# rendeirolab/stainx

Hardware: AMD Instinct MI355X
Metric: megapixels/sec Macenko transform, 64x3x512x512 fp32; max-abs vs torch CPU (higher is better)
Workload: dtype f32; 1 GPU; Macenko reference-mode transform, 64x3x512x512 fp32 per GPU (BASELINE configs[1]); tiles_per_gpu=64, height=512, width=512, input_batches_rotated=2, parallelism=tiles sharded over 1 GPU(s), no collective

## Files before the change

### stainx_amd/csrc/macenko_twopass.hpp

```cpp
#pragma once

namespace sx {
namespace macenko {

constexpr int kPriorSweeps = 4;
constexpr int kPriorUnitsMax = kGroupThreads / 4 * kPriorSweeps;
constexpr int kQueue2 = 512;
constexpr float kSpecSigmasConc = 5.0f, kSpecThresholdScale = 1.0f;
constexpr float kSpecSigmas = 5.0f;
constexpr float kSpecEffFar = 2.0f, kSpecEffNear = 1.0f;
__device__ __forceinline__ float spec_eff(const Geometry& g) { return g.prior_step_q16 >= (8u << 16) ? g.spec_eff_far : g.spec_eff_near; }
constexpr float kSpecKw = 0.10f, kSpecKx = 1.3e-3f;
constexpr float kSpecRot = 0.30f;
constexpr uint32_t kSpecSlow = 1u, kSpecHazard = 2u;
constexpr int kMaxSegments = 256;

constexpr int kRowBelowA = 0, kRowAboveA = 1, kRowBelowB = 2, kRowAboveB = 3, kRowConc = 4, kRowW = 8;
struct alignas(128) PriorRecord {
    float a0[3], a1[3], an[3];
    float rows[16][4];
    float kw, kx;
    float cmax[4];
    int32_t mode;
    int32_t min_first;
// ... 2 lines not shown

struct alignas(64) FusedTile {
    uint32_t a_done;
    uint32_t s_done;
    uint32_t ncand[kSlots];
    uint32_t pad[10];
};
constexpr int kXcds = 8;
struct alignas(64) FusedQueue {
    uint32_t ticket;
    uint32_t pad[15];
};
struct FusedSched {
    FusedQueue queue[kXcds];
};
static_assert(sizeof(FusedTile) == kFusedTileBytes && sizeof(FusedSched) <= kFusedSchedBytes, "workspace layout");


typedef unsigned int sx_u4 __attribute__((ext_vector_type(4)));
__device__ __forceinline__ uint32_t ld_agent(const uint32_t* p) { return __hip_atomic_load(p, __ATOMIC_RELAXED, __HIP_MEMORY_SCOPE_AGENT); }
__device__ __forceinline__ int32_t ld_agent(const int32_t* p) { return __hip_atomic_load(p, __ATOMIC_RELAXED, __HIP_MEMORY_SCOPE_AGENT); }
__device__ __forceinline__ float ld_agent(const float* p) { return __uint_as_float(__hip_atomic_load(reinterpret_cast<const uint32_t*>(p), __ATOMIC_RELAXED, __HIP_MEMORY_SCOPE_AGENT)); }
__device__ __forceinline__ double ld_agent(const double* p) {
    return __longlong_as_double((long long)__hip_atomic_load(reinterpret_cast<const unsigned long long*>(p), __ATOMIC_RELAXED, __HIP_MEMORY_SCOPE_AGENT));
}
__device__ __forceinline__ void st_agent(uint32_t* p, uint32_t v) { __hip_atomic_store(p, v, __ATOMIC_RELAXED, __HIP_MEMORY_SCOPE_AGENT); }
__device__ __forceinline__ void st_agent(float* p, float v) { __hip_atomic_store(reinterpret_cast<uint32_t*>(p), __float_as_uint(v), __ATOMIC_RELAXED, __HIP_MEMORY_SCOPE_AGENT); }
__device__ __forceinline__ void st_agent(double* p, double v) {
    __hip_atomic_store(reinterpret_cast<unsigned long long*>(p), (unsigned long long)__double_as_longlong(v), __ATOMIC_RELAXED, __HIP_MEMORY_SCOPE_AGENT);
}
__device__ __forceinline__ void drain_stores() { asm volatile("s_waitcnt vmcnt(0)" ::: "memory"); }

constexpr int kPriorBins = 2048;
constexpr float kOpenExponent = 30.0f;
constexpr float kOpenNear = 16.0f;
struct alignas(16) PriorScratch {
    double red[kGroupThreads / kWave][kPartial];
    double mom[kMoments];
    uint32_t hist[4][kPriorBins];
    uint32_t od16[kPriorSweeps][6][kGroupThreads];
    uint32_t n_kept, n_all, hazard, r_max;
    float frame[9];
    float bdir[4][2];
    float bkey[4], blevel[4];
    float cthr[4];
    uint32_t cmax[4];
    uint32_t open;
};

__device__ __forceinline__ uint32_t prior_pick_bin(const uint32_t* hist, uint32_t rank) {
    constexpr int kPer = kPriorBins / kWave;
    static_assert(kPer <= kWave, "second level: one bin per lane");
    const int lane = (int)lane_id();
    uint32_t mine = 0;
#pragma unroll 8
    for (int i = 0; i < kPer; ++i) mine += hist[kPer * lane + i];
    const uint32_t incl = wave_scan_u32(mine);
    const uint64_t over = __ballot(incl > rank);
    const int owner = over ? (__ffsll((long long)over) - 1) : (kWave - 1);
    const uint32_t r = rank - (uint32_t)__builtin_amdgcn_readlane((int)(incl - mine), owner);
    const uint32_t h = lane < kPer ? hist[kPer * owner + lane] : 0u;
    const uint32_t incl2 = wave_scan_u32(h);
    const uint64_t over2 = __ballot(lane < kPer && incl2 > r);
    const int sub = over2 ? (__ffsll((long long)over2) - 1) : (kPer - 1);
    return (uint32_t)(kPer * owner + sub);
}

__device__ __forceinline__ float wave_total_f32(float x) {
    auto step = [](float v, auto mover) { return v + __uint_as_float(mover(__float_as_uint(v))); };
    x = step(x, [](uint32_t b) { return dpp_move<0x111, 0xF>(0u, b); });
    x = step(x, [](uint32_t b) { return dpp_move<0x112, 0xF>(0u, b); });
    x = step(x, [](uint32_t b) { return dpp_move<0x114, 0xF>(0u, b); });
    x = step(x, [](uint32_t b) { return dpp_move<0x118, 0xF>(0u, b); });
    x = step(x, [](uint32_t b) { return dpp_move<0x142, 0xA>(0u, b); });
    x = step(x, [](uint32_t b) { return dpp_move<0x143, 0xC>(0u, b); });
    return x;
}

// ... 20 lines not shown
}
template <typename T>
__device__ __forceinline__ void prior_densities(const float (&u)[3][4], float (&od)[4][3]) {
#pragma unroll
    for (int i = 0; i < 4; ++i)
#pragma unroll
        for (int c = 0; c < 3; ++c) od[i][c] = optical_density<T>(u[c][i]);
}

template <typename T, bool kVec, bool kInter>
__global__ __launch_bounds__(kGroupThreads) void prior_kernel(const T* __restrict__ images, Geometry g, Workspace ws) {
    __shared__ PriorScratch sh;
    const int tile = blockIdx.x, tid = threadIdx.x, wave = tid / kWave;
    const uint32_t lane = lane_id();
    GroupState& st = ws.state[tile];
    PriorRecord* pr = &ws.prior[tile];
    const T* img = images + (int64_t)tile * 3 * g.pixels;
    SX_STAMP(st, 0);
    if (tid < kSlots) {
        put(&st.ncand[tid], 0u);
        put(&st.below[tid], 0u);
        put(&st.ncand_seen[tid], 0u);
        put(&st.over_count[tid], 0u);
    }
    if (tid < 2) put(&st.phi_pub[tid], 0ull);
    if ((g.fused || g.dense) && tid < (int)(sizeof(FusedTile) / 4)) put(reinterpret_cast<uint32_t*>(&ws.ftile[tile]) + tid, 0u);
    if (g.fused && tile == 0 && tid >= 32 && tid < 32 + kXcds) put(&ws.fsched->queue[tid - 32].ticket, 0u);
    if (tid == 0) {
        put(&st.fell_back, 0u);
        put(&st.spec, 0u);
        sh.n_kept = sh.n_all = sh.hazard = sh.open = sh.r_max = 0;
        sh.cmax[0] = sh.cmax[1] = sh.cmax[2] = sh.cmax[3] = 0;
    }
    for (int i = tid; i < 4 * kPriorBins; i += kGroupThreads) (&sh.hist[0][0])[i] = 0;

    {
        float m[kPartial];
#pragma unroll
        for (int k = 0; k < kPartial; ++k) m[k] = 0.0f;
        float raw[kPriorSweeps][3][4];
        bool have_quad[kPriorSweeps];
#pragma unroll
        for (int s = 0; s < kPriorSweeps; ++s) have_quad[s] = prior_fetch<T, kVec, kInter>(img, g, s, raw[s]);
#pragma unroll
        for (int s = 0; s < kPriorSweeps; ++s) {
            float od[4][3];
            prior_densities<T>(raw[s], od);
            const bool have = have_quad[s];
#pragma unroll
            for (int q = 0; q < 6; ++q) {
                const int e = 2 * q;
                typedef __fp16 fp16x2 __attribute__((ext_vector_type(2)));
                const fp16x2 h = __builtin_amdgcn_cvt_pkrtz(od[e / 3][e % 3], od[(e + 1) / 3][(e + 1) % 3]);
                sh.od16[s][q][tid] = __builtin_bit_cast(uint32_t, h);
            }
#pragma unroll
            for (int i = 0; i < 4; ++i) {
                const float* o = od[i];
                const float keep = (have && od_selected(o, false)) ? 1.0f : 0.0f;
                const float k0 = keep * o[0], k1 = keep * o[1], k2 = keep * o[2];
                m[0] += keep;
                m[1] += k0;
                m[2] += k1;
                m[3] += k2;
                m[4] = fmaf(k0, o[0], m[4]);
                m[5] = fmaf(k0, o[1], m[5]);
                m[6] = fmaf(k0, o[2], m[6]);
// ... 73 lines not shown
            if (have) have_bits |= 1u << s;
#pragma unroll
            for (int i = 0; i < 4; ++i) {
                const float* o = od[i];
                t0[s][i] = fmaf(o[2], fr[2], fmaf(o[1], fr[1], o[0] * fr[0]));
                t1[s][i] = fmaf(o[2], fr[5], fmaf(o[1], fr[4], o[0] * fr[3]));
                if (have) {
                    r_max = fmaxf(r_max, fabsf(t0[s][i]) + fabsf(t1[s][i]));
                    if (i == s) ++all;
                    if (od_selected(o, false)) {
                        if (!(t1[s][i] - 0.05f * fabsf(t0[s][i]) > 0.0f)) haz = 1;
                        if (i == s) {
                            ++cnt;
                            sub_kept |= 1u << s;
                        }
                    }
                }
            }
        }
        cnt = wave_total_u32(cnt);
        all = wave_total_u32(all);
        const uint32_t rm = wave_max_u32(__float_as_uint(r_max));
        const uint64_t hz = __ballot(haz != 0);
        if (lane == 0) {
            if (cnt) atomicAdd(&sh.n_kept, cnt);
            atomicAdd(&sh.n_all, all);
            atomicMax(&sh.r_max, rm);
            if (hz) atomicOr(&sh.hazard, 1u);
        }
#pragma unroll
        for (int s = 0; s < kPriorSweeps; ++s)
            if ((sub_kept >> s) & 1u) {
                const float d = diamond_angle(t1[s][s], t0[s][s]);
                atomicAdd(&sh.hist[0][min((uint32_t)fmaxf(d * (float)(kPriorBins / 2), 0.0f), (uint32_t)(kPriorBins - 1))], 1u);
            }
    }
    __syncthreads();
    SX_STAMP(st, 4);
    if (sh.hazard) {
        give_up();
        return;
    }
    const int mv = (int)sh.n_kept, ms = (int)sh.n_all;
    if (wave < 4) {
        const float f = wave < 2 ? 0.01f : 0.99f;
        const float n_eff = fmaxf((float)mv * (spec_eff(g) / 4.0f), 4.0f);
        const float sd = sqrtf(f * (1.0f - f) / n_eff);
        const bool upper = (wave & 1) != 0;
        const float level = upper ? f + g.spec_sigmas * sd : f - g.spec_sigmas * sd;
        const bool open = mv < 16 || (upper ? level >= 1.0f : level <= 0.0f);
        const float pos = fminf(fmaxf(level, 0.0f), 1.0f) * (float)max(mv - 1, 0);
        const uint32_t rank = (uint32_t)min(max((int)(upper ? ceilf(pos) : floorf(pos)), 0), max(mv - 1, 0));
        const uint32_t b = prior_pick_bin(sh.hist[0], rank);
        if (lane == 0) {
            sh.bkey[wave] = upper ? (float)(b + 1) * (2.0f / kPriorBins) : (float)b * (2.0f / kPriorBins);
            sh.blevel[wave] = fminf(fmaxf(level, 0.0f), 1.0f) * n_eff;
            if (open) atomicOr(&sh.open, 1u << wave);
        }
    }
    __syncthreads();
    if (tid < 4) {
        const bool upper = (tid & 1) != 0, open = ((sh.open >> tid) & 1u) != 0, partner_open = ((sh.open >> (tid ^ 1)) & 1u) != 0;
        float d = sh.bkey[tid];
        if (open) {
            const float other = sh.bkey[tid ^ 1];
            const float n_eff = fmaxf((float)mv * (spec_eff(g) / 4.0f), 4.0f);
            const float m_near = upper ? n_eff - sh.blevel[tid ^ 1] : sh.blevel[tid ^ 1];
            const bool tight = !partner_open && m_near >= kOpenNear;
            const float w = fminf(fmaxf((kOpenExponent - 0.01f * n_eff) / fmaxf(m_near, 1.0f), 0.25f), 1.0f);
            d = !tight ? (upper ? 1.98f : 0.02f) : (upper ? d + w * fmaxf(d - other, 0.0f) + 2.0f / kPriorBins : d - w * fmaxf(other - d, 0.0f) - 2.0f / kPriorBins);
        }
        d = fminf(fmaxf(d, 0.02f), 1.98f);
        float c, s;
        direction_from_key(float_key(d), c, s);
        sh.bdir[tid][0] = c;
        sh.bdir[tid][1] = s;
    }
    __syncthreads();
    SX_STAMP(st, 5);
    float bd[4][2];
#pragma unroll
    for (int q = 0; q < 4; ++q) {
        bd[q][0] = sh.bdir[q][0];
        bd[q][1] = sh.bdir[q][1];
    }
    const float lo_c = bd[0][0] + bd[1][0], lo_s = bd[0][1] + bd[1][1], hi_c = bd[2][0] + bd[3][0], hi_s = bd[2][1] + bd[3][1];
    const bool min_first = (fr[0] * lo_c + fr[3] * lo_s) * __builtin_amdgcn_rsqf(lo_c * lo_c + lo_s * lo_s) > (fr[0] * hi_c + fr[3] * hi_s) * __builtin_amdgcn_rsqf(hi_c * hi_c + hi_s * hi_s);
    float cu[4][2];
    {
        const int slot_perp_high = min_first ? 0 : 1, slot_perp_low = 1 - slot_perp_high;
#pragma unroll
        for (int e = 0; e < 2; ++e) {
            cu[2 * slot_perp_high + e][0] = bd[2 + e][1];
            cu[2 * slot_perp_high + e][1] = -bd[2 + e][0];
            cu[2 * slot_perp_low + e][0] = -bd[e][1];
            cu[2 * slot_perp_low + e][1] = bd[e][0];
        }
    }
    const float r_max = __uint_as_float(sh.r_max);
    const float c_scale = r_max > 0.0f ? (float)kPriorBins / r_max : 0.0f;
    for (int i = tid; i < kPriorBins; i += kGroupThreads) sh.hist[0][i] = 0;
    __syncthreads();
#pragma unroll
    for (int q = 0; q < 4; ++q) {
        float k_max = 0.0f;
#pragma unroll
        for (int s = 0; s < kPriorSweeps; ++s)
            if ((have_bits >> s) & 1u) {
                const float k = fmaf(cu[q][0], t0[s][s], cu[q][1] * t1[s][s]);
                k_max = fmaxf(k_max, k);
                atomicAdd(&sh.hist[q][min((uint32_t)fmaxf(k * c_scale, 0.0f), (uint32_t)(kPriorBins - 1))], 1u);
            }
        const uint32_t km = wave_max_u32(__float_as_uint(k_max));
        if (lane == 0) atomicMax(&sh.cmax[q], km);
    }
    __syncthreads();
    SX_STAMP(st, 6);
    if (wave < 4) {
        const float n_eff = fmaxf((float)ms * (spec_eff(g) / 4.0f), 4.0f);
        const float level = 0.99f - g.spec_sigmas_conc * sqrtf(0.99f * 0.01f / n_eff);
        const uint32_t rank = (uint32_t)max((int)floorf(fmaxf(level, 0.0f) * (float)max(ms - 1, 0)), 0);
        const uint32_t b = prior_pick_bin(sh.hist[wave], rank);
        if (lane == 0) sh.cthr[wave] = (level > 0.0f && b > 0) ? g.spec_tscale * (float)b * (r_max / (float)kPriorBins) : -__builtin_huge_valf();
    }
    __syncthreads();
    if (tid < 9) {
        const float* a0 = &sh.frame[0];
        const float* a1 = &sh.frame[3];
        const float* an = &sh.frame[6];
        const uint32_t open = sh.open;
        float row[4] = {0.0f, 0.0f, 0.0f, 0.0f};
#pragma unroll
        for (int q = 0; q < 4; ++q) {
            if (tid == q && ((open >> q) & 1u) == 0) {
#pragma unroll
                for (int c = 0; c < 3; ++c) row[c] = bd[q][0] * a1[c] - bd[q][1] * a0[c];
            }
            if (tid == kRowConc + q) {
#pragma unroll
                for (int c = 0; c < 3; ++c) row[c] = cu[q][0] * a0[c] + cu[q][1] * a1[c];
                row[3] = sh.cthr[q] > -1e30f ? -sh.cthr[q] : 60000.0f;
            }
        }
        if (tid == kRowW) {
#pragma unroll
            for (int c = 0; c < 3; ++c) row[c] = an[c];
        }
#pragma unroll
        for (int c = 0; c < 4; ++c) put(&pr->rows[tid][c], __half2float(__float2half_rn(row[c])));
    } else if (tid < 16) {
#pragma unroll
        for (int c = 0; c < 4; ++c) put(&pr->rows[tid][c], 0.0f);
    }
    if (tid == 0) {
#pragma unroll
        for (int i = 0; i < 3; ++i) {
            put(&pr->a0[i], sh.frame[i]);
            put(&pr->a1[i], sh.frame[3 + i]);
            put(&pr->an[i], sh.frame[6 + i]);
        }
        put(&pr->kw, g.spec_kw);
        put(&pr->kx, kSpecKx);
#pragma unroll
        for (int q = 0; q < 4; ++q) put(&pr->cmax[q], __uint_as_float(sh.cmax[q]));
        put(&pr->mode, 0);
        put(&pr->min_first, min_first ? 1 : 0);
        put(&pr->open, sh.open);
    }
    SX_STAMP(st, 7);
}

template <int TPB> struct PassAScratch {
    StatsScratch<TPB> stats;
    uint32_t queue[TPB / kWave][4][kQueue2];
    uint32_t below[2];
};

__device__ __forceinline__ void write_records(const uint32_t (*__restrict__ queue)[kQueue2], uint32_t n, uint32_t (&have)[kSlots], float* __restrict__ cand_tile, const Geometry& g, uint32_t seg_base, uint32_t* __restrict__ over_count) {
    const uint32_t cap2 = g.cap2, seg_cap = g.seg_cap, over_base = (uint32_t)g.n_seg * g.seg_cap;
    for (uint32_t i0 = 0; i0 < n; i0 += kWave) {
        const uint32_t i = i0 + lane_id();
        uint4 rec = make_uint4(0u, 0u, 0u, 0u);
        if (i < n) rec = make_uint4(queue[0][i], queue[1][i], queue[2][i], queue[3][i]);
#pragma unroll
        for (int s = 0; s < kSlots; ++s) {
            const bool has = ((rec.w >> s) & 1u) != 0;
            const uint64_t mask = __builtin_amdgcn_ballot_w64(has);
// ... 253 lines not shown
    }
    double kept_total = 0.0;
#pragma unroll
    for (int w = 0; w < TPB / kWave; ++w) kept_total += ss->red[w][0];
    if (__builtin_expect(kept_total < 3.0, 0)) {
        if (!tile_has_three_kept_witnesses<T, TPB, kInter>(img, g.pixels)) {
            stats_item_all_pixels<T, V, TPB, kInter>(img, g.pixels, p_begin, p_end, ws.partial_all + item * kPartial, ss);
            if constexpr (kFused) __builtin_amdgcn_fence(__ATOMIC_RELEASE, "agent");
        }
    }
    if constexpr (kFused) {
        drain_stores();
        __syncthreads();
        if (threadIdx.x == 0) __hip_atomic_fetch_add(&ws.ftile[tile].a_done, 1u, __ATOMIC_RELAXED, __HIP_MEMORY_SCOPE_AGENT);
    }
}

template <typename T, int V, bool kInter = false, bool kDense = false>
__global__ __launch_bounds__(kStreamThreads, (Codable<T, V, kInter>::value ? 4 : 1)) void pass_a_kernel(const T* __restrict__ images, Geometry g, Workspace ws) {
    __shared__ PassAScratch<kStreamThreads> sh;
    __shared__ LevelTables<T> tb;
    tb.fill();
    if constexpr (Codable<T, V, kInter>::value) {
        if (g.code_epoch != 0u) {
            __shared__ CodeTable<T, 2> ct;
            ct.fill();
            pass_a_item<T, V, kStreamThreads, kInter, kDense, true>(images, g, ws, blockIdx.x / g.blocks_per_tile, blockIdx.x % g.blocks_per_tile, blockIdx.x, &sh, tb, &ct);
            return;
        }
    }
    pass_a_item<T, V, kStreamThreads, kInter, kDense>(images, g, ws, blockIdx.x / g.blocks_per_tile, blockIdx.x % g.blocks_per_tile, blockIdx.x, &sh, tb);
}

struct alignas(16) SlotScratch {
    TileScratch t;
    uint32_t keys[kLdsKeys];
    float vecs[6], pinv[6], he[6];
    double check[8];
    uint32_t lo, hi, n_list, bin, rank_in_bin, result, range_first, range_last, bin_count;
    int ok, use_all;
    unsigned long long n_sel;
    uint32_t seg_prefix[kMaxSegments + 1], seg_total, seg_overflow, over_n;
    uint32_t dense_n;
    uint32_t own_key;
    int partner_ok;
    uint32_t k_floor, k_ceil, n_under;
};

__device__ __forceinline__ void segment_prefix(SlotScratch* sh, const Geometry& g, const Workspace& ws, int tile, int slot) {
    if (threadIdx.x < kWave) {
        const uint32_t* counts = ws.seg_count + ((size_t)tile * kSlots + slot) * g.n_seg;
        uint32_t c[4], sum = 0, raw = 0;
#pragma unroll
        for (int u = 0; u < 4; ++u) {
            const int k = 4 * (int)threadIdx.x + u;
            const uint32_t v = k < g.n_seg ? get(&counts[k]) : 0u;
            raw += v;
            c[u] = min(v, g.seg_cap);
            sum += c[u];
        }
        const uint32_t incl = wave_scan_u32(sum);
        uint32_t run = incl - sum;
#pragma unroll
        for (int u = 0; u < 4; ++u) {
            const int k = 4 * (int)threadIdx.x + u;
            if (k <= g.n_seg) sh->seg_prefix[k] = run;
            run += c[u];
        }
        const uint32_t total_raw = wave_total_u32(raw);
        if (threadIdx.x == kWave - 1) {
            const uint32_t spilled = get(&ws.state[tile].over_count[slot]);
            sh->seg_prefix[g.n_seg] = incl;
            sh->seg_total = total_raw;
            sh->over_n = min(spilled, g.over_cap);
            sh->seg_overflow = spilled > g.over_cap ? 1u : 0u;
        }
    }
}

// ... 60 lines not shown
#pragma unroll
    for (int u = 0; u < kPre; ++u) {
        const uint32_t i = threadIdx.x + (uint32_t)u * blockDim.x;
        if (i < n) fn(i, pf.od[u]);
    }
    constexpr int kFlight = 4;
    for (uint32_t i0 = threadIdx.x + (uint32_t)kPre * blockDim.x; i0 < n; i0 += blockDim.x * kFlight) {
        float od[kFlight][3];
#pragma unroll
        for (int u = 0; u < kFlight; ++u) {
            const sx_u4 rec = __builtin_amdgcn_raw_buffer_load_b128(rsrc, (int)((i0 + (uint32_t)u * blockDim.x) * 16u), 0, 0);
#pragma unroll
            for (int c = 0; c < 3; ++c) od[u][c] = __uint_as_float(rec[c]);
        }
#pragma unroll
        for (int u = 0; u < kFlight; ++u) {
            const uint32_t i = i0 + (uint32_t)u * blockDim.x;
            if (i < n) fn(i, od[u]);
        }
    }
}
__device__ __forceinline__ void dense_count(SlotScratch* sh, const Geometry& g, const Workspace& ws, int tile, int slot) {
    if (threadIdx.x == kWave - 1) {
        const uint32_t n_raw = get(&ws.ftile[tile].ncand[slot]);
        sh->seg_total = n_raw;
        sh->dense_n = min(n_raw, g.fused_cap);
        sh->over_n = 0;
        sh->seg_overflow = n_raw > g.fused_cap ? 1u : 0u;
    }
}

__device__ __forceinline__ uint32_t slot_key(const SlotScratch* sh, const uint32_t* __restrict__ spill, uint32_t i) { return i < (uint32_t)kLdsKeys ? sh->keys[i] : get(&spill[i - kLdsKeys]); }

__device__ __forceinline__ void select_prepare(SlotScratch* sh) {
    if (threadIdx.x == 0) {
        sh->lo = 0xFFFFFFFFu;
        sh->hi = 0u;
        sh->n_list = 0;
        sh->result = 0;
        sh->n_under = 0;
    }
    for (int i = threadIdx.x; i < 512; i += blockDim.x) (&sh->t.hist_c[0][0])[i] = 0;
}
__device__ __forceinline__ void publish_range(SlotScratch* sh, uint32_t mn, uint32_t mx) {
    mn = wave_min_u32(mn);
    mx = wave_max_u32(mx);
    if (lane_id() == 0 && mn != 0xFFFFFFFFu) {
        atomicMin(&sh->lo, mn);
        atomicMax(&sh->hi, mx);
    }
}

__device__ uint32_t select_slot_keys(SlotScratch* sh, const uint32_t* __restrict__ spill, uint32_t n, uint32_t rank, bool level0_filled, unsigned long long* dbg = nullptr, uint32_t k_floor = 0u, uint32_t k_ceil = 0xFFFFFFFFu) {
    const uint32_t lane = lane_id();
    const int wave = threadIdx.x / kWave;
    const uint32_t share = ((n + blockDim.x - 1) / blockDim.x) | 1u, i_begin = min(threadIdx.x * share, n), i_end = min(i_begin + share, n);
    const uint32_t lo = max(sh->lo, k_floor), hi = max(min(sh->hi, k_ceil), lo);
    double origin = bin_origin_for(lo), scale = bin_scale_for(lo, hi);
    uint32_t k_first = k_floor, k_last = 0xFFFFFFFFu, want = rank;
    uint32_t picked = 0;
    bool by_bin = false;
    uint32_t* hist = sh->t.hist_c[0];
    for (int level = 0; level < 2; ++level) {
        if (level > 0 || !level0_filled) {
            for (uint32_t i = i_begin; i < i_end; ++i) {
                const uint32_t k = slot_key(sh, spill, i);
                if (k >= k_first && k <= k_last) atomicAdd(&hist[bin_of(k, origin, scale)], 1u);
            }
            __syncthreads();
        }
        if (dbg && threadIdx.x == 0) dbg[level] = (unsigned long long)wall_clock64();
        if (wave == 0) {
            uint32_t b, rb;
            scan_pick32(hist, want, b, rb);
            if (lane == 0) {
                const uint32_t in_bin = hist[b];
                sh->bin = b;
                sh->rank_in_bin = rb;
                sh->bin_count = in_bin;
                if (in_bin > (uint32_t)kShortList || level == 1) {
                    uint32_t first, last;
                    bin_key_range(b, origin, scale, first, last);
                    sh->range_first = max(first, k_first);
                    sh->range_last = min(last, k_last);
                }
            }
        }
        __syncthreads();
        want = sh->rank_in_bin;
        picked = sh->bin;
        const uint32_t in_bin = sh->bin_count;
// ... 15 lines not shown
        const uint32_t k = slot_key(sh, spill, i);
        if (k >= k_first && k <= k_last && (!by_bin || bin_of(k, origin, scale) == picked)) {
            const uint32_t at = atomicAdd(&sh->n_list, 1u);
            if (at < (uint32_t)(2 * kSample)) list[at] = k;
        }
    }
    __syncthreads();
    if (dbg && threadIdx.x == 0) dbg[2] = (unsigned long long)wall_clock64();
    const uint32_t n_list = sh->n_list;
    if (__builtin_expect(n_list <= (uint32_t)kShortList, 1)) {
        rank_pick(list, n_list, want, threadIdx.x, blockDim.x, &sh->result);
        __syncthreads();
        return sh->result;
    }
    if (n_list <= (uint32_t)(2 * kSample)) return radix_select_stream((unsigned long long)n_list, (unsigned long long)want, [list](unsigned long long i, uint32_t& k) { k = list[i]; return true; }, &sh->t);
    return radix_select_stream((unsigned long long)n, (unsigned long long)rank, [sh, spill, k_floor](unsigned long long i, uint32_t& k) { k = slot_key(sh, spill, (uint32_t)i); return k >= k_floor; }, &sh->t);
}

__device__ inline void frame_coordinates(const PriorRecord* pr, const float x[3], float out[3]) {
    const float f00 = pr->a0[0], f10 = pr->a0[1], f20 = pr->a0[2];
    const float f01 = pr->a1[0], f11 = pr->a1[1], f21 = pr->a1[2];
    const float f02 = pr->an[0], f12 = pr->an[1], f22 = pr->an[2];
    const float c00 = f11 * f22 - f12 * f21, c01 = f12 * f20 - f10 * f22, c02 = f10 * f21 - f11 * f20;
    const float det = f00 * c00 + f01 * c01 + f02 * c02;
    const float inv = det != 0.0f ? __builtin_amdgcn_rcpf(det) : 0.0f;
    const float i00 = c00 * inv, i01 = (f02 * f21 - f01 * f22) * inv, i02 = (f01 * f12 - f02 * f11) * inv;
    const float i10 = c01 * inv, i11 = (f00 * f22 - f02 * f20) * inv, i12 = (f02 * f10 - f00 * f12) * inv;
    const float i20 = c02 * inv, i21 = (f01 * f20 - f00 * f21) * inv, i22 = (f00 * f11 - f01 * f10) * inv;
    out[0] = i00 * x[0] + i01 * x[1] + i02 * x[2];
    out[1] = i10 * x[0] + i11 * x[1] + i12 * x[2];
    out[2] = i20 * x[0] + i21 * x[1] + i22 * x[2];
}

template <typename T>
__device__ void exact_plane(const Geometry& g, const Workspace& ws, int tile, SlotScratch* sh) {
    const int64_t first = (int64_t)tile * g.blocks_per_tile;
    if (threadIdx.x < kPartial) {
        double running = 0.0;
        for (int64_t b0 = 0; b0 < g.blocks_per_tile; b0 += 16) {
            double part[16];
#pragma unroll
            for (int u = 0; u < 16; ++u) part[u] = b0 + u < g.blocks_per_tile ? get(&ws.partial[(first + b0 + u) * kPartial + threadIdx.x]) : 0.0;
#pragma unroll
            for (int u = 0; u < 16; ++u)
                if (b0 + u < g.blocks_per_tile) running += part[u];
        }
        sh->t.mom[threadIdx.x] = running;
    }
    if (threadIdx.x == kPartial) sh->t.mom[kPartial] = (double)g.pixels;
    if (threadIdx.x > kPartial && threadIdx.x < kMoments) sh->t.mom[threadIdx.x] = 0.0;
    __syncthreads();
    if (__builtin_expect(sh->t.mom[0] < 3.0, 0)) {
        __syncthreads();
        if (threadIdx.x < kPartial) {
            double running = 0.0;
            for (int64_t b = 0; b < g.blocks_per_tile; ++b) running += get(&ws.partial_all[(first + b) * kPartial + threadIdx.x]);
            sh->t.mom[kPartial + threadIdx.x] = running;
        }
        __syncthreads();
    }
    if (threadIdx.x < 2) {
        double cov[9];
        bool use_all;
        unsigned long long n_sel;
        float vecs[6];
        plane_from_moments<true>(sh->t.mom, true, cov, vecs, use_all, n_sel);
        if (threadIdx.x == 0) {
#pragma unroll
            for (int i = 0; i < 6; ++i) sh->vecs[i] = vecs[i];
            sh->use_all = use_all ? 1 : 0;
            sh->n_sel = n_sel;
            if ((blockIdx.x & 1) == 0) {
                GroupState& st = ws.state[tile];
#pragma unroll
                for (int i = 0; i < 6; ++i) {
                    put(&st.vecs[i], vecs[i]);
                    put(&st.rec[0].coef[i], vecs[i]);
                }
#pragma unroll
                for (int k = 0; k < kMoments; ++k) put(&st.mom[k], sh->t.mom[k]);
#pragma unroll
                for (int i = 0; i < 9; ++i) put(&st.cov[i], cov[i]);
                put(&st.use_all, use_all ? 1 : 0);
                put(&st.rec[0].use_all, use_all ? 1 : 0);
                put(&st.n_sel, n_sel);
            }
        }
    }
    __syncthreads();
}

__device__ inline bool phi_slot_check(const PriorRecord* pr, const float (&v)[6], int j, double (&check)[8], float rot_limit) {
    float m0[3], m1[3];
    const float v0[3] = {v[0], v[2], v[4]}, v1[3] = {v[1], v[3], v[5]};
    frame_coordinates(pr, v0, m0);
    frame_coordinates(pr, v1, m1);
    const float r00 = m0[0], r01 = m0[1], r10 = m1[0], r11 = m1[1], nu0 = m0[2], nu1 = m1[2];
    const float det = r00 * r11 - r01 * r10;
    const float nu = __builtin_amdgcn_sqrtf(nu0 * nu0 + nu1 * nu1);
    const float stretch = __builtin_amdgcn_sqrtf(r00 * r00 + r01 * r01 + r10 * r10 + r11 * r11);
    const float kw = get(&pr->kw), kx = get(&pr->kx);
    bool good = det > 0.9f && stretch < 1.6f && r00 > 0.8f && r11 > 0.8f && fabsf(r01) + fabsf(r10) < rot_limit && kx >= 1.2e-3f;
    {
        const float a1_min = fminf(pr->a1[0], fminf(pr->a1[1], pr->a1[2]));
        const float a0_max = fmaxf(fabsf(pr->a0[0]), fmaxf(fabsf(pr->a0[1]), fabsf(pr->a0[2])));
        const float an_max = fmaxf(fabsf(pr->an[0]), fmaxf(fabsf(pr->an[1]), fabsf(pr->an[2])));
        if (!(r11 * a1_min > 1.05f * (fabsf(r10) * a0_max + nu * an_max))) good = false;
    }
    const uint32_t open = get(&pr->open);
#pragma unroll
    for (int e = 0; e < 2; ++e) {
        const float* row = pr->rows[2 * j + e];
        float gq[3];
        frame_coordinates(pr, row, gq);
        const float dx = gq[1], dy = -gq[0];
        const float mx = r00 * dx + r01 * dy, my = r10 * dx + r11 * dy;
        const bool is_open = ((open >> (2 * j + e)) & 1u) != 0;
        check[e] = is_open ? (e ? 2.0 : 0.0) : (double)diamond_angle(my, mx);
        check[2 + e] = is_open ? 1.0 : 0.0;
        if (!is_open) {
            const float dn = __builtin_amdgcn_sqrtf(dx * dx + dy * dy);
            if (!(my - 0.04f * fabsf(mx) > 0.0f)) good = false;
            if (!(fmaxf(fabsf(row[0]), fmaxf(fabsf(row[1]), fabsf(row[2]))) <= 1.05f)) good = false;
            if (!(nu * stretch * dn * 1.05f <= (kw - fabsf(gq[2])) * det)) good = false;
        }
    }
    if (!(check[1] > check[0])) good = false;
    return good;
}

__device__ inline bool conc_slot_check(const PriorRecord* pr, const float (&pinv)[6], int j, double& theta_out, float& hi_out) {
    const float p[3] = {pinv[3 * j], pinv[3 * j + 1], pinv[3 * j + 2]};
    float gq[3], g1[3], g2[3];
    frame_coordinates(pr, p, gq);
    const float* row1 = pr->rows[kRowConc + 2 * j];
    const float* row2 = pr->rows[kRowConc + 2 * j + 1];
    frame_coordinates(pr, row1, g1);
    frame_coordinates(pr, row2, g2);
    const float u1x = g1[0], u1y = g1[1], t1 = -row1[3], u2x = g2[0], u2y = g2[1], t2 = -row2[3];
    const float det = u1x * u2y - u1y * u2x;
    const float kw = get(&pr->kw), kx = get(&pr->kx);
    if (!(fabsf(det) > 1e-7f)) return false;
    const float inv = __builtin_amdgcn_rcpf(det);
    const float alpha = (gq[0] * u2y - gq[1] * u2x) * inv, beta = (u1x * gq[1] - u1y * gq[0]) * inv;
    const float l1 = fabsf(p[0]) + fabsf(p[1]) + fabsf(p[2]);
    const float rmax = fmaxf(fmaxf(fabsf(row1[0]), fmaxf(fabsf(row1[1]), fabsf(row1[2]))), fmaxf(fabsf(row2[0]), fmaxf(fabsf(row2[1]), fabsf(row2[2]))));
    const bool good = alpha >= 1e-5f * l1 && beta >= 1e-5f * l1 && rmax <= 1.05f && kx >= 1.2e-3f &&
                      (alpha + beta) * kw >= 1.05f * (alpha * fabsf(g1[2]) + beta * fabsf(g2[2]) + fabsf(gq[2])) && (alpha + beta) * (kx - 1.1e-3f) >= 3e-6f * l1 && t1 < 1e30f && t2 < 1e30f;
    theta_out = (double)alpha * (double)t1 + (double)beta * (double)t2;
    const float span = alpha * fmaxf(get(&pr->cmax[2 * j]) - t1, 0.0f) + beta * fmaxf(get(&pr->cmax[2 * j + 1]) - t2, 0.0f);
    hi_out = (float)theta_out + fmaxf(1.25f * span, 1e-3f * fabsf((float)theta_out) + 1e-6f);
    return good;
}

template <typename T, bool kDense = false>
__global__ __launch_bounds__(kGroupThreads) void estimate_stage_kernel(const T* __restrict__ images, Geometry g, Workspace ws, const float* __restrict__ target_max_conc,
                                                                       uint32_t* __restrict__ key_scratch) {
    __shared__ SlotScratch sh;
    const int tile = blockIdx.x >> 1, j = blockIdx.x & 1, slot = 2 + j;
    uint32_t* keep = key_scratch ? key_scratch + ((size_t)tile * 3 + j) * (size_t)g.pixels * (sizeof(T) >= 4 ? sizeof(T) / 4 : 1) : nullptr;
    GroupState& st = ws.state[tile];
    const PriorRecord* pr = &ws.prior[tile];
    const uint32_t below = get(&st.below[j]), spec = get(&st.spec);
    const int mode = get(&pr->mode);
    const bool stamps = j == 0;
    if (stamps) SX_STAMP(st, 8);
    const float* c0 = ws.cand_od + ((size_t)tile * kSlots + j) * 3 * g.cap2;
    const size_t spill_words = kDense ? (g.fused_cap > (uint32_t)kLdsKeys ? g.fused_cap - kLdsKeys : 0u) : (g.cap2 > (uint32_t)kLdsKeys ? g.cap2 - kLdsKeys : 0u);
    uint32_t* const spill_area = kDense ? ws.dense_spill : ws.key_spill;
    const uint4* rec_tile = ws.cand_rec + (size_t)__builtin_amdgcn_readfirstlane(tile) * kSlots * g.fused_cap;
    const auto rsrc_phi = __builtin_amdgcn_make_buffer_rsrc(const_cast<uint4*>(rec_tile + (size_t)__builtin_amdgcn_readfirstlane(j) * g.fused_cap), 0, (int)(g.fused_cap * 16u), 0x00020000);
    const auto rsrc_conc = __builtin_amdgcn_make_buffer_rsrc(const_cast<uint4*>(rec_tile + (size_t)__builtin_amdgcn_readfirstlane(slot) * g.fused_cap), 0, (int)(g.fused_cap * 16u), 0x00020000);
    float v[6];
    bool use_all;
    unsigned long long rank_other;
    {
        CandPrefetch<8> pf;
        if constexpr (kDense) prefetch_candidates_dense(pf, rsrc_phi); else prefetch_candidates(pf, g, c0);
        select_prepare(&sh);
        if constexpr (kDense) dense_count(&sh, g, ws, tile, j); else segment_prefix(&sh, g, ws, tile, j);
        exact_plane<T>(g, ws, tile, &sh);
#pragma unroll
        for (int i = 0; i < 6; ++i) v[i] = sh.vecs[i];
        if (stamps) SX_STAMP(st, 9);
        const uint32_t n = kDense ? sh.dense_n : sh.seg_prefix[g.n_seg] + sh.over_n, n_raw = sh.seg_total;
        use_all = sh.use_all != 0;
        const unsigned long long n_sel = sh.n_sel;
        const unsigned long long rank = nearest_rank_index(j ? 99.0 : 1.0, n_sel);
        rank_other = nearest_rank_index(j ? 1.0 : 99.0, n_sel);
        bool ok = mode == 0 && (spec & (kSpecSlow | kSpecHazard)) == 0 && !use_all && !g.spec_fail && sh.seg_overflow == 0 && rank >= below && rank - below < n;
        uint32_t* spill = spill_area + ((size_t)tile * kSlots + j) * spill_words;
        uint32_t answer = 0, why = 1u;
        if (ok) {
            uint32_t mn = 0xFFFFFFFFu, mx = 0u;
            auto phi_key_of = [&](uint32_t i, const float (&od)[3]) {
                const uint32_t k = angle_key(od, v);
                mn = min(mn, k);
                mx = max(mx, k);
                if (i < (uint32_t)kLdsKeys) sh.keys[i] = k; else put(&spill[i - kLdsKeys], k);
            };
            if constexpr (kDense) for_each_candidate_dense(pf, n, rsrc_phi, phi_key_of); else for_each_candidate(pf, &sh, g, c0, phi_key_of);
            publish_range(&sh, mn, mx);
            if (threadIdx.x == kGroupThreads - 1) sh.ok = phi_slot_check(pr, v, j, sh.check, g.spec_rot) ? 1 : 0;
            __syncthreads();
            if (stamps) SX_STAMP(st, 10);
            ok = sh.ok != 0;
            why = 2u;
        }
        if (ok) {
            answer = select_slot_keys(&sh, spill, n, (uint32_t)(rank - below), false);
            const float a = key_float(answer);
            const double slack = 4e-6;
            if (sh.check[2] == 0.0 && !((double)a >= sh.check[0] + slack)) ok = false;
            if (sh.check[3] == 0.0 && !((double)a <= sh.check[1] - slack)) ok = false;
            why = 3u;
        }
        if (!ok) {
            __syncthreads();
            if (threadIdx.x == 0) {
                atomicOr(&st.fell_back, 1u << j);
                atomicOr(&st.spec, (sh.seg_overflow ? 4u : why) << (8 + 4 * j));
                atomicAdd(&ws.state[0].slow_slots, 1u);
            }
            reset_scratch(&sh.t);
            answer = select_whole_group<T>(images, g, tile, j, rank, v, use_all, &sh.t, keep);
        }
        if (threadIdx.x == 0) {
            put(&st.phi_key[j], answer);
            put(&st.rank[j], rank);
            put(&st.ncand_seen[j], mode == 0 ? n_raw : 0u);
            __hip_atomic_store(&st.phi_pub[j], (1ull << 32) | (unsigned long long)answer, __ATOMIC_RELAXED, __HIP_MEMORY_SCOPE_AGENT);
            sh.own_key = answer;
        }
        if (stamps) SX_STAMP(st, 11);
    }
    if (stamps) SX_STAMP(st, 12);
    const float* c1 = ws.cand_od + ((size_t)tile * kSlots + slot) * 3 * g.cap2;
    CandPrefetch<12> pf;
    if constexpr (kDense) prefetch_candidates_dense(pf, rsrc_conc); else prefetch_candidates(pf, g, c1);
    __syncthreads();
    select_prepare(&sh);
    if constexpr (kDense) dense_count(&sh, g, ws, tile, slot); else segment_prefix(&sh, g, ws, tile, slot);
    auto vectors_and_check = [&](uint32_t partner_key) {
        float he[6], pinv[6];
        const uint32_t key0 = j == 0 ? sh.own_key : partner_key, key1 = j == 0 ? partner_key : sh.own_key;
        stain_vectors_and_pinv(v, key0, key1, he, pinv);
#pragma unroll
        for (int i = 0; i < 6; ++i) {
            sh.pinv[i] = pinv[i];
            sh.he[i] = he[i];
        }
        double theta = 0.0;
        float hi = 0.0f;
        const bool good = mode == 0 && conc_slot_check(pr, pinv, j, theta, hi);
        sh.check[0] = theta;
        sh.ok = good ? 1 : 0;
        const double bound = theta + 4e-6 * fabs(theta) + 1e-7;
        uint32_t kf = float_key((float)bound);
        if ((double)key_float(kf) > bound && kf > 0u) --kf;
        sh.k_floor = good ? kf : 0u;
        sh.k_ceil = good ? max(float_key(hi), kf) : 0xFFFFFFFFu;
    };
    if (threadIdx.x == kWave) {
        unsigned long long granule = 0;
        for (int spin = 0; spin < (1 << 16); ++spin) {
            granule = __hip_atomic_load(&st.phi_pub[1 - j], __ATOMIC_RELAXED, __HIP_MEMORY_SCOPE_AGENT);
            if ((granule >> 32) == 1ull) break;
            __builtin_amdgcn_s_sleep(4);
        }
        sh.partner_ok = (granule >> 32) == 1ull ? 1 : 0;
        if (sh.partner_ok) vectors_and_check((uint32_t)granule);
    }
    __syncthreads();
    if (__builtin_expect(sh.partner_ok == 0, 0)) {
        reset_scratch(&sh.t);
        const uint32_t partner_key = select_whole_group<T>(images, g, tile, 1 - j, rank_other, v, use_all, &sh.t, keep);
        __syncthreads();
        select_prepare(&sh);
        if (threadIdx.x == kWave) vectors_and_check(partner_key);
        __syncthreads();
    }
    float pinv[6];
#pragma unroll
    for (int i = 0; i < 6; ++i) pinv[i] = sh.pinv[i];
    const unsigned long long n_all = (unsigned long long)g.pixels;
    const unsigned long long k99 = nearest_rank_index(99.0, n_all);
    const uint32_t n = kDense ? sh.dense_n : sh.seg_prefix[g.n_seg] + sh.over_n, n_raw = sh.seg_total;
    if (stamps) SX_STAMP(st, 13);
    const unsigned long long outside = n_all - (unsigned long long)n;
    bool ok = mode == 0 && (spec & (kSpecSlow | kSpecHazard)) == 0 && !g.spec_fail && sh.seg_overflow == 0 && k99 >= outside && n > 0;
    uint32_t why = ok && sh.ok == 0 ? 2u : 1u;
    ok = ok && sh.ok != 0;
    uint32_t* spill = spill_area + ((size_t)tile * kSlots + slot) * spill_words;
    uint32_t answer = 0;
    if (ok) {
        const uint32_t k_floor = sh.k_floor, k_ceil = sh.k_ceil;
        uint32_t mn = 0xFFFFFFFFu, mx = 0u, under = 0u;
        auto conc_key_of = [&](uint32_t i, const float (&od)[3]) {
            float ca, cb;
            concentration(od, pinv, ca, cb);
            const uint32_t k = float_key(j ? cb : ca);
            mn = min(mn, k);
            mx = max(mx, k);
            under += k < k_floor ? 1u : 0u;
            if (i < (uint32_t)kLdsKeys) sh.keys[i] = k; else put(&spill[i - kLdsKeys], k);
        };
        if constexpr (kDense) for_each_candidate_dense(pf, n, rsrc_conc, conc_key_of); else for_each_candidate(pf, &sh, g, c1, conc_key_of);
        publish_range(&sh, mn, mx);
        under = wave_total_u32(under);
        if (lane_id() == 0 && under) atomicAdd(&sh.n_under, under);
        __syncthreads();
        if (stamps) SX_STAMP(st, 14);
        const unsigned long long rank_in = k99 - outside;
        const uint32_t n_under = sh.n_under;
        why = 3u;
        if (rank_in < n_under) {
            ok = false;
        } else {
            answer = select_slot_keys(&sh, spill, n, (uint32_t)(rank_in - n_under), false, nullptr, k_floor, k_ceil);
            const double a = (double)key_float(answer), theta = sh.check[0];
            if (!(a >= theta + 4e-6 * fabs(theta) + 1e-7)) ok = false;
        }
    }
    if (!ok) {
        __syncthreads();
        if (threadIdx.x == 0) {
            atomicOr(&st.fell_back, 1u << slot);
            atomicOr(&st.spec, (sh.seg_overflow ? 4u : why) << (8 + 4 * slot));
            atomicAdd(&ws.state[0].slow_slots, 1u);
        }
        reset_scratch(&sh.t);
        answer = select_whole_group<T>(images, g, tile, slot, k99, pinv, true, &sh.t, keep);
    }
    if (threadIdx.x == 0) {
        const float mc = key_float(answer);
        put(&st.max_c[j], mc);
        put(&st.rank[slot], k99);
        put(&st.ncand_seen[slot], mode == 0 ? n_raw : 0u);
        StageRecord* rec = &st.rec[2];
        put(&rec->scale[j], target_max_conc[j] / mc);
        if (j == 0) {
#pragma unroll
            for (int i = 0; i < 6; ++i) {
                put(&rec->coef[i], pinv[i]);
                put(&st.pinv[i], pinv[i]);
                put(&st.he[i], sh.he[i]);
            }
        }
    }
    if (stamps) SX_STAMP(st, 15);
}

// ... 3 lines not shown
```

Measured before the change: 112,000 megapixels/s.

## Build level-0 selection histograms during key generation using prior-derived bin ranges

Key ranges for the phi and concentration selections are now derived in advance: from the prior record's frame and boundary directions for phi, and from the check bounds k_floor/k_ceil for concentration. This lets the level-0 histogram be filled while the keys are generated, so the first select pass no longer rescans the keys and the min/max range reductions are dropped. The prior record is also copied into LDS for the slot checks. The prior kernel gets a separate angle histogram plane, which removes a clear-and-sync step, and it writes its rows per wave. The risk is that the predicted ranges can be looser than the true min/max, which gives coarser bins, and it adds more LDS per block.

```diff
diff --git a/stainx_amd/csrc/macenko_twopass.hpp b/stainx_amd/csrc/macenko_twopass.hpp
--- a/stainx_amd/csrc/macenko_twopass.hpp
+++ b/stainx_amd/csrc/macenko_twopass.hpp
@@ -58,18 +58,18 @@
 __device__ __forceinline__ void drain_stores() { asm volatile("s_waitcnt vmcnt(0)" ::: "memory"); }
 
 constexpr int kPriorBins = 2048;
+constexpr int kPriorAnglePlane = 4;
 constexpr float kOpenExponent = 30.0f;
 constexpr float kOpenNear = 16.0f;
 struct alignas(16) PriorScratch {
     double red[kGroupThreads / kWave][kPartial];
     double mom[kMoments];
-    uint32_t hist[4][kPriorBins];
+    uint32_t hist[5][kPriorBins];
     uint32_t od16[kPriorSweeps][6][kGroupThreads];
     uint32_t n_kept, n_all, hazard, r_max;
     float frame[9];
     float bdir[4][2];
     float bkey[4], blevel[4];
-    float cthr[4];
     uint32_t cmax[4];
     uint32_t open;
 };
@@ -156,7 +156,7 @@
         sh.n_kept = sh.n_all = sh.hazard = sh.open = sh.r_max = 0;
         sh.cmax[0] = sh.cmax[1] = sh.cmax[2] = sh.cmax[3] = 0;
     }
-    for (int i = tid; i < 4 * kPriorBins; i += kGroupThreads) (&sh.hist[0][0])[i] = 0;
+    for (int i = tid; i < 5 * kPriorBins; i += kGroupThreads) (&sh.hist[0][0])[i] = 0;
 
     {
         float m[kPartial];
@@ -296,7 +296,7 @@
         for (int s = 0; s < kPriorSweeps; ++s)
             if ((sub_kept >> s) & 1u) {
                 const float d = diamond_angle(t1[s][s], t0[s][s]);
-                atomicAdd(&sh.hist[0][min((uint32_t)fmaxf(d * (float)(kPriorBins / 2), 0.0f), (uint32_t)(kPriorBins - 1))], 1u);
+                atomicAdd(&sh.hist[kPriorAnglePlane][min((uint32_t)fmaxf(d * (float)(kPriorBins / 2), 0.0f), (uint32_t)(kPriorBins - 1))], 1u);
             }
     }
     __syncthreads();
@@ -315,7 +315,7 @@
         const bool open = mv < 16 || (upper ? level >= 1.0f : level <= 0.0f);
         const float pos = fminf(fmaxf(level, 0.0f), 1.0f) * (float)max(mv - 1, 0);
         const uint32_t rank = (uint32_t)min(max((int)(upper ? ceilf(pos) : floorf(pos)), 0), max(mv - 1, 0));
-        const uint32_t b = prior_pick_bin(sh.hist[0], rank);
+        const uint32_t b = prior_pick_bin(sh.hist[kPriorAnglePlane], rank);
         if (lane == 0) {
             sh.bkey[wave] = upper ? (float)(b + 1) * (2.0f / kPriorBins) : (float)b * (2.0f / kPriorBins);
             sh.blevel[wave] = fminf(fmaxf(level, 0.0f), 1.0f) * n_eff;
@@ -363,8 +363,6 @@
     }
     const float r_max = __uint_as_float(sh.r_max);
     const float c_scale = r_max > 0.0f ? (float)kPriorBins / r_max : 0.0f;
-    for (int i = tid; i < kPriorBins; i += kGroupThreads) sh.hist[0][i] = 0;
-    __syncthreads();
 #pragma unroll
     for (int q = 0; q < 4; ++q) {
         float k_max = 0.0f;
@@ -380,43 +378,46 @@
     }
     __syncthreads();
     SX_STAMP(st, 6);
+    const float* a0 = &sh.frame[0];
+    const float* a1 = &sh.frame[3];
+    const float* an = &sh.frame[6];
     if (wave < 4) {
         const float n_eff = fmaxf((float)ms * (spec_eff(g) / 4.0f), 4.0f);
         const float level = 0.99f - g.spec_sigmas_conc * sqrtf(0.99f * 0.01f / n_eff);
         const uint32_t rank = (uint32_t)max((int)floorf(fmaxf(level, 0.0f) * (float)max(ms - 1, 0)), 0);
         const uint32_t b = prior_pick_bin(sh.hist[wave], rank);
-        if (lane == 0) sh.cthr[wave] = (level > 0.0f && b > 0) ? g.spec_tscale * (float)b * (r_max / (float)kPriorBins) : -__builtin_huge_valf();
-    }
-    __syncthreads();
-    if (tid < 9) {
-        const float* a0 = &sh.frame[0];
-        const float* a1 = &sh.frame[3];
-        const float* an = &sh.frame[6];
+        if (lane == 0) {
+            const float cthr = (level > 0.0f && b > 0) ? g.spec_tscale * (float)b * (r_max / (float)kPriorBins) : -__builtin_huge_valf();
+            float row[4] = {0.0f, 0.0f, 0.0f, 0.0f};
+#pragma unroll
+            for (int q = 0; q < 4; ++q)
+                if (wave == q) {
+#pragma unroll
+                    for (int c = 0; c < 3; ++c) row[c] = cu[q][0] * a0[c] + cu[q][1] * a1[c];
+                }
+            row[3] = cthr > -1e30f ? -cthr : 60000.0f;
+#pragma unroll
+            for (int c = 0; c < 4; ++c) put(&pr->rows[kRowConc + wave][c], __half2float(__float2half_rn(row[c])));
+        }
+    } else if (wave == 4) {
         const uint32_t open = sh.open;
         float row[4] = {0.0f, 0.0f, 0.0f, 0.0f};
 #pragma unroll
         for (int q = 0; q < 4; ++q) {
-            if (tid == q && ((open >> q) & 1u) == 0) {
+            if ((int)lane == q && ((open >> q) & 1u) == 0) {
 #pragma unroll
                 for (int c = 0; c < 3; ++c) row[c] = bd[q][0] * a1[c] - bd[q][1] * a0[c];
             }
-            if (tid == kRowConc + q) {
-#pragma unroll
-                for (int c = 0; c < 3; ++c) row[c] = cu[q][0] * a0[c] + cu[q][1] * a1[c];
-                row[3] = sh.cthr[q] > -1e30f ? -sh.cthr[q] : 60000.0f;
-            }
-        }
-        if (tid == kRowW) {
+        }
+        if ((int)lane == kRowW) {
 #pragma unroll
             for (int c = 0; c < 3; ++c) row[c] = an[c];
         }
-#pragma unroll
-        for (int c = 0; c < 4; ++c) put(&pr->rows[tid][c], __half2float(__float2half_rn(row[c])));
-    } else if (tid < 16) {
-#pragma unroll
-        for (int c = 0; c < 4; ++c) put(&pr->rows[tid][c], 0.0f);
-    }
-    if (tid == 0) {
+        if (lane < 16 && (lane < (uint32_t)kRowConc || lane >= (uint32_t)kRowW)) {
+#pragma unroll
+            for (int c = 0; c < 4; ++c) put(&pr->rows[lane][c], __half2float(__float2half_rn(row[c])));
+        }
+    } else if (wave == 5 && lane == 0) {
 #pragma unroll
         for (int i = 0; i < 3; ++i) {
             put(&pr->a0[i], sh.frame[i]);
@@ -736,7 +737,11 @@
     pass_a_item<T, V, kStreamThreads, kInter, kDense>(images, g, ws, blockIdx.x / g.blocks_per_tile, blockIdx.x % g.blocks_per_tile, blockIdx.x, &sh, tb);
 }
 
-struct alignas(16) SlotScratch {
+struct PhiBinSetup {
+    float inv[9];
+    float dir[2][2];
+};
+struct alignas(128) SlotScratch {
     TileScratch t;
     uint32_t keys[kLdsKeys];
     float vecs[6], pinv[6], he[6];
@@ -749,6 +754,8 @@
     uint32_t own_key;
     int partner_ok;
     uint32_t k_floor, k_ceil, n_under;
+    PriorRecord prior;
+    PhiBinSetup phi_bins;
 };
 
 __device__ __forceinline__ void segment_prefix(SlotScratch* sh, const Geometry& g, const Workspace& ws, int tile, int slot) {
@@ -875,31 +882,30 @@
 
 __device__ __forceinline__ uint32_t slot_key(const SlotScratch* sh, const uint32_t* __restrict__ spill, uint32_t i) { return i < (uint32_t)kLdsKeys ? sh->keys[i] : get(&spill[i - kLdsKeys]); }
 
-__device__ __forceinline__ void select_prepare(SlotScratch* sh) {
+__device__ __forceinline__ void select_prepare(SlotScratch* sh, bool keep_range = false) {
     if (threadIdx.x == 0) {
-        sh->lo = 0xFFFFFFFFu;
-        sh->hi = 0u;
+        if (!keep_range) {
+            sh->lo = 0xFFFFFFFFu;
+            sh->hi = 0u;
+        }
         sh->n_list = 0;
         sh->result = 0;
         sh->n_under = 0;
     }
     for (int i = threadIdx.x; i < 512; i += blockDim.x) (&sh->t.hist_c[0][0])[i] = 0;
 }
-__device__ __forceinline__ void publish_range(SlotScratch* sh, uint32_t mn, uint32_t mx) {
-    mn = wave_min_u32(mn);
-    mx = wave_max_u32(mx);
-    if (lane_id() == 0 && mn != 0xFFFFFFFFu) {
-        atomicMin(&sh->lo, mn);
-        atomicMax(&sh->hi, mx);
-    }
+__device__ __forceinline__ void slot_bins(const SlotScratch* sh, uint32_t k_floor, uint32_t k_ceil, double& origin, double& scale) {
+    const uint32_t lo = max(sh->lo, k_floor), hi = max(min(sh->hi, k_ceil), lo);
+    origin = bin_origin_for(lo);
+    scale = bin_scale_for(lo, hi);
 }
 
 __device__ uint32_t select_slot_keys(SlotScratch* sh, const uint32_t* __restrict__ spill, uint32_t n, uint32_t rank, bool level0_filled, unsigned long long* dbg = nullptr, uint32_t k_floor = 0u, uint32_t k_ceil = 0xFFFFFFFFu) {
     const uint32_t lane = lane_id();
     const int wave = threadIdx.x / kWave;
     const uint32_t share = ((n + blockDim.x - 1) / blockDim.x) | 1u, i_begin = min(threadIdx.x * share, n), i_end = min(i_begin + share, n);
-    const uint32_t lo = max(sh->lo, k_floor), hi = max(min(sh->hi, k_ceil), lo);
-    double origin = bin_origin_for(lo), scale = bin_scale_for(lo, hi);
+    double origin, scale;
+    slot_bins(sh, k_floor, k_ceil, origin, scale);
     uint32_t k_first = k_floor, k_last = 0xFFFFFFFFu, want = rank;
     uint32_t picked = 0;
     bool by_bin = false;
@@ -981,8 +987,7 @@
     out[2] = i20 * x[0] + i21 * x[1] + i22 * x[2];
 }
 
-template <typename T>
-__device__ void exact_plane(const Geometry& g, const Workspace& ws, int tile, SlotScratch* sh) {
+__device__ __forceinline__ void exact_moments(const Geometry& g, const Workspace& ws, int tile, SlotScratch* sh) {
     const int64_t first = (int64_t)tile * g.blocks_per_tile;
     if (threadIdx.x < kPartial) {
         double running = 0.0;
@@ -998,6 +1003,10 @@
     }
     if (threadIdx.x == kPartial) sh->t.mom[kPartial] = (double)g.pixels;
     if (threadIdx.x > kPartial && threadIdx.x < kMoments) sh->t.mom[threadIdx.x] = 0.0;
+}
+template <typename T, class Tail>
+__device__ void exact_plane(const Geometry& g, const Workspace& ws, int tile, SlotScratch* sh, Tail tail) {
+    const int64_t first = (int64_t)tile * g.blocks_per_tile;
     __syncthreads();
     if (__builtin_expect(sh->t.mom[0] < 3.0, 0)) {
         __syncthreads();
@@ -1034,6 +1043,7 @@
                 put(&st.rec[0].use_all, use_all ? 1 : 0);
                 put(&st.n_sel, n_sel);
             }
+            tail(vecs);
         }
     }
     __syncthreads();
@@ -1076,6 +1086,56 @@
     }
     if (!(check[1] > check[0])) good = false;
     return good;
+}
+
+__device__ inline void phi_bin_setup(const PriorRecord* pr, int j, PhiBinSetup* out) {
+    const float f00 = get(&pr->a0[0]), f10 = get(&pr->a0[1]), f20 = get(&pr->a0[2]);
+    const float f01 = get(&pr->a1[0]), f11 = get(&pr->a1[1]), f21 = get(&pr->a1[2]);
+    const float f02 = get(&pr->an[0]), f12 = get(&pr->an[1]), f22 = get(&pr->an[2]);
+    const uint32_t open = get(&pr->open);
+    const int perp_high = get(&pr->min_first) ? 0 : 1;
+    float row[2][3];
+    bool stand_in[2];
+#pragma unroll
+    for (int e = 0; e < 2; ++e) {
+        stand_in[e] = ((open >> (2 * j + e)) & 1u) != 0;
+        const float* r = pr->rows[stand_in[e] ? kRowConc + 2 * (j ? perp_high : 1 - perp_high) + e : 2 * j + e];
+#pragma unroll
+        for (int c = 0; c < 3; ++c) row[e][c] = get(&r[c]);
+    }
+    const float c00 = f11 * f22 - f12 * f21, c01 = f12 * f20 - f10 * f22, c02 = f10 * f21 - f11 * f20;
+    const float det = f00 * c00 + f01 * c01 + f02 * c02;
+    const float s = det != 0.0f ? __builtin_amdgcn_rcpf(det) : 0.0f;
+    const float inv[9] = {c00 * s, (f02 * f21 - f01 * f22) * s, (f01 * f12 - f02 * f11) * s,
+                          c01 * s, (f00 * f22 - f02 * f20) * s, (f02 * f10 - f00 * f12) * s,
+                          c02 * s, (f01 * f20 - f00 * f21) * s, (f00 * f11 - f01 * f10) * s};
+#pragma unroll
+    for (int i = 0; i < 9; ++i) out->inv[i] = inv[i];
+#pragma unroll
+    for (int e = 0; e < 2; ++e) {
+        const float g0 = inv[0] * row[e][0] + inv[1] * row[e][1] + inv[2] * row[e][2], g1 = inv[3] * row[e][0] + inv[4] * row[e][1] + inv[5] * row[e][2];
+        const bool flip = stand_in[e] && j == 1;
+        out->dir[e][0] = flip ? -g1 : g1;
+        out->dir[e][1] = flip ? g0 : -g0;
+    }
+}
+__device__ inline void phi_bin_range(const PhiBinSetup* su, const float (&v)[6], uint32_t& lo, uint32_t& hi) {
+    const float* inv = su->inv;
+    const float r00 = inv[0] * v[0] + inv[1] * v[2] + inv[2] * v[4], r01 = inv[3] * v[0] + inv[4] * v[2] + inv[5] * v[4];
+    const float r10 = inv[0] * v[1] + inv[1] * v[3] + inv[2] * v[5], r11 = inv[3] * v[1] + inv[4] * v[3] + inv[5] * v[5];
+    float key[2];
+#pragma unroll
+    for (int e = 0; e < 2; ++e) {
+        const float dx = su->dir[e][0], dy = su->dir[e][1];
+        const float mx = r00 * dx + r01 * dy, my = r10 * dx + r11 * dy;
+        key[e] = my > 0.0f ? diamond_angle(my, mx) : (e ? 2.0f : 0.0f);
+    }
+    if (!(key[1] > key[0])) {
+        key[0] = 0.0f;
+        key[1] = 2.0f;
+    }
+    lo = float_key(key[0]);
+    hi = float_key(key[1]);
 }
 
 __device__ inline bool conc_slot_check(const PriorRecord* pr, const float (&pinv)[6], int j, double& theta_out, float& hi_out) {
@@ -1124,11 +1184,19 @@
     bool use_all;
     unsigned long long rank_other;
     {
+        exact_moments(g, ws, tile, &sh);
+        if (threadIdx.x >= kGroupThreads - (int)(sizeof(PriorRecord) / 4)) {
+            const int w = threadIdx.x - (kGroupThreads - (int)(sizeof(PriorRecord) / 4));
+            reinterpret_cast<uint32_t*>(&sh.prior)[w] = get(reinterpret_cast<const uint32_t*>(pr) + w);
+        }
+        if (threadIdx.x == kWave && mode == 0) phi_bin_setup(pr, j, &sh.phi_bins);
         CandPrefetch<8> pf;
         if constexpr (kDense) prefetch_candidates_dense(pf, rsrc_phi); else prefetch_candidates(pf, g, c0);
         select_prepare(&sh);
         if constexpr (kDense) dense_count(&sh, g, ws, tile, j); else segment_prefix(&sh, g, ws, tile, j);
-        exact_plane<T>(g, ws, tile, &sh);
+        exact_plane<T>(g, ws, tile, &sh, [&](const float (&vecs)[6]) {
+            if (mode == 0) phi_bin_range(&sh.phi_bins, vecs, sh.lo, sh.hi);
+        });
 #pragma unroll
         for (int i = 0; i < 6; ++i) v[i] = sh.vecs[i];
         if (stamps) SX_STAMP(st, 9);
@@ -1141,23 +1209,23 @@
         uint32_t* spill = spill_area + ((size_t)tile * kSlots + j) * spill_words;
         uint32_t answer = 0, why = 1u;
         if (ok) {
-            uint32_t mn = 0xFFFFFFFFu, mx = 0u;
+            double origin, scale;
+            slot_bins(&sh, 0u, 0xFFFFFFFFu, origin, scale);
+            uint32_t* hist = sh.t.hist_c[0];
             auto phi_key_of = [&](uint32_t i, const float (&od)[3]) {
                 const uint32_t k = angle_key(od, v);
-                mn = min(mn, k);
-                mx = max(mx, k);
                 if (i < (uint32_t)kLdsKeys) sh.keys[i] = k; else put(&spill[i - kLdsKeys], k);
+                atomicAdd(&hist[bin_of(k, origin, scale)], 1u);
             };
             if constexpr (kDense) for_each_candidate_dense(pf, n, rsrc_phi, phi_key_of); else for_each_candidate(pf, &sh, g, c0, phi_key_of);
-            publish_range(&sh, mn, mx);
-            if (threadIdx.x == kGroupThreads - 1) sh.ok = phi_slot_check(pr, v, j, sh.check, g.spec_rot) ? 1 : 0;
+            if (threadIdx.x == kGroupThreads - 1) sh.ok = phi_slot_check(&sh.prior, v, j, sh.check, g.spec_rot) ? 1 : 0;
             __syncthreads();
             if (stamps) SX_STAMP(st, 10);
             ok = sh.ok != 0;
             why = 2u;
         }
         if (ok) {
-            answer = select_slot_keys(&sh, spill, n, (uint32_t)(rank - below), false);
+            answer = select_slot_keys(&sh, spill, n, (uint32_t)(rank - below), true);
             const float a = key_float(answer);
             const double slack = 4e-6;
             if (sh.check[2] == 0.0 && !((double)a >= sh.check[0] + slack)) ok = false;
@@ -1188,7 +1256,7 @@
     CandPrefetch<12> pf;
     if constexpr (kDense) prefetch_candidates_dense(pf, rsrc_conc); else prefetch_candidates(pf, g, c1);
     __syncthreads();
-    select_prepare(&sh);
+    select_prepare(&sh, true);
     if constexpr (kDense) dense_count(&sh, g, ws, tile, slot); else segment_prefix(&sh, g, ws, tile, slot);
     auto vectors_and_check = [&](uint32_t partner_key) {
         float he[6], pinv[6];
@@ -1201,7 +1269,7 @@
         }
         double theta = 0.0;
         float hi = 0.0f;
-        const bool good = mode == 0 && conc_slot_check(pr, pinv, j, theta, hi);
+        const bool good = mode == 0 && conc_slot_check(&sh.prior, pinv, j, theta, hi);
         sh.check[0] = theta;
         sh.ok = good ? 1 : 0;
         const double bound = theta + 4e-6 * fabs(theta) + 1e-7;
@@ -1209,6 +1277,8 @@
         if ((double)key_float(kf) > bound && kf > 0u) --kf;
         sh.k_floor = good ? kf : 0u;
         sh.k_ceil = good ? max(float_key(hi), kf) : 0xFFFFFFFFu;
+        sh.lo = sh.k_floor;
+        sh.hi = sh.k_ceil;
     };
     if (threadIdx.x == kWave) {
         unsigned long long granule = 0;
@@ -1225,7 +1295,7 @@
         reset_scratch(&sh.t);
         const uint32_t partner_key = select_whole_group<T>(images, g, tile, 1 - j, rank_other, v, use_all, &sh.t, keep);
         __syncthreads();
-        select_prepare(&sh);
+        select_prepare(&sh, true);
         if (threadIdx.x == kWave) vectors_and_check(partner_key);
         __syncthreads();
     }
@@ -1244,18 +1314,18 @@
     uint32_t answer = 0;
     if (ok) {
         const uint32_t k_floor = sh.k_floor, k_ceil = sh.k_ceil;
-        uint32_t mn = 0xFFFFFFFFu, mx = 0u, under = 0u;
+        uint32_t under = 0u;
+        double origin, scale;
+        slot_bins(&sh, k_floor, k_ceil, origin, scale);
+        uint32_t* hist = sh.t.hist_c[0];
         auto conc_key_of = [&](uint32_t i, const float (&od)[3]) {
             float ca, cb;
             concentration(od, pinv, ca, cb);
             const uint32_t k = float_key(j ? cb : ca);
-            mn = min(mn, k);
-            mx = max(mx, k);
-            under += k < k_floor ? 1u : 0u;
             if (i < (uint32_t)kLdsKeys) sh.keys[i] = k; else put(&spill[i - kLdsKeys], k);
+            if (k < k_floor) ++under; else atomicAdd(&hist[bin_of(k, origin, scale)], 1u);
         };
         if constexpr (kDense) for_each_candidate_dense(pf, n, rsrc_conc, conc_key_of); else for_each_candidate(pf, &sh, g, c1, conc_key_of);
-        publish_range(&sh, mn, mx);
         under = wave_total_u32(under);
         if (lane_id() == 0 && under) atomicAdd(&sh.n_under, under);
         __syncthreads();
@@ -1266,7 +1336,7 @@
         if (rank_in < n_under) {
             ok = false;
         } else {
-            answer = select_slot_keys(&sh, spill, n, (uint32_t)(rank_in - n_under), false, nullptr, k_floor, k_ceil);
+            answer = select_slot_keys(&sh, spill, n, (uint32_t)(rank_in - n_under), true, nullptr, k_floor, k_ceil);
             const double a = (double)key_float(answer), theta = sh.check[0];
             if (!(a >= theta + 4e-6 * fabs(theta) + 1e-7)) ok = false;
         }
```

Measured after the change: 114,400 megapixels/s (median of 6 runs). 2.1% higher.
